# ribal-aladeeb/reinforcement-learning-2048

Hardware: AMD Instinct MI355X
Metric: 2048 env steps/sec + DQN updates/sec at 64k parallel boards, 1→8 MI355X (higher is better)
Workload: dtype u8

## Files before the change

### reinforcement-learning-2048_amd/csrc/g2048_conv64.hip

```cpp
#include <hip/hip_runtime.h>
#include <math.h>
#include <stdint.h>
#include <stdlib.h>

#include <mutex>
#include <unordered_map>

#include "../../include/g2048.h"
#include "g2048_board.hpp"
#include "g2048_common.hpp"

namespace {

typedef double d4 __attribute__((ext_vector_type(4)));

constexpr int NT = 256;
constexpr int TB = 16;
constexpr int XS = 17;
constexpr int DSB = 66;
constexpr int DPL = TB * DSB;
constexpr int HS = 258;
constexpr int H3S = 66;
constexpr int MAX_WG = 256;

constexpr int P_W1 = 0, P_B1 = 256, P_W2 = 320, P_B2 = 16704, P_F1 = 16768, P_FB1 = 33152,
              P_F2 = 33216, P_FB2 = 33472, P_N = 33476;
constexpr int SLAB = P_N + 4;
constexpr int FC_D2_LO = P_F1 / 2, FC_D2_HI = P_N / 2 + 1, FC_D2 = FC_D2_HI - FC_D2_LO;
constexpr int SHADOW_MIN_GRID = (FC_D2 + 63) / 64;
static_assert(P_F1 % 2 == 0 && P_N % 2 == 0 && SLAB % 2 == 0, "double2 ranges");
constexpr int PACK = 16384;
constexpr int PACKU = 9 * 4096;
constexpr int O_U_ON = 0, O_F1_ON = PACKU, O_U_TG = PACKU + PACK, O_F1_TG = 2 * PACKU + PACK,
              O_F1B = 2 * PACKU + 2 * PACK, O_UB = 2 * PACKU + 3 * PACK,
              PACK_ALL = 3 * PACKU + 3 * PACK, PACK_FWD = PACKU + PACK;
static_assert(PACK_ALL % 256 == 0 && PACK_FWD % 256 == 0, "pack grid");
constexpr int WS_STEP = PACK_ALL, WS_SLAB = PACK_ALL + 32;

#ifdef G2048_PHASE_PROF
__device__ unsigned long long g_cphase[32];
__shared__ unsigned long long g_lph[24];
#define CPHASE_INIT()                                                     \
    do {                                                                  \
        if (threadIdx.x == 0) {                                           \
            for (int k_ = 0; k_ < 23; ++k_) g_lph[k_] = 0ull;             \
            g_lph[23] = __builtin_amdgcn_s_memtime();                     \
        }                                                                 \
    } while (0)
#define CPHASE(k)                                                         \
    do {                                                                  \
        if (__builtin_amdgcn_readfirstlane(threadIdx.x) < 64) {           \
            const unsigned long long n_ = __builtin_amdgcn_s_memtime();   \
            if ((k) >= 0) g_lph[(k) < 0 ? 0 : (k)] += n_ - g_lph[23];     \
            g_lph[23] = n_;                                               \
        }                                                                 \
    } while (0)
#define CPHASE_FLUSH()                                                    \
    do {                                                                  \
        if (blockIdx.x == 0 && threadIdx.x == 0)                          \
            for (int k_ = 0; k_ < 23; ++k_) atomicAdd(&g_cphase[k_], g_lph[k_]); \
    } while (0)
#else
#define CPHASE_INIT()
#define CPHASE(k)
#define CPHASE_FLUSH()
#endif

typedef __attribute__((address_space(1))) const double gdouble;
__device__ __forceinline__ const gdouble* opaque(const double* p) {
    const gdouble* g = (const gdouble*)p;
    asm volatile("" : "+s"(g));
    return g;
}

__device__ __forceinline__ d4 mfma(double a, double b, d4 c) {
    return __builtin_amdgcn_mfma_f64_16x16x4f64(a, b, c, 0, 0, 0);
}

struct Net {
    const double *w1, *b1, *w2, *b2, *f1, *fb1, *f2, *fb2;
};

struct Packed {
    const double *u, *pf1;
};

struct SmallW {
    double w1[256], b1[64], b2[64], fb1[64], f2[256], fb2[4];
};

struct alignas(16) Smem {
    double x[TB * XS];
    double d[9 * DPL];
    double h2[TB * HS];
    double h3[TB * H3S];
    SmallW sw[2];
    double q[TB * 4];
    double q2[TB * 4];
    double y[TB];
    double r[TB];
    double dq[TB];
    double loss[TB];
    double f2p[4 * TB * 4];
    float disc[TB];
    int act[TB];
};

__device__ __forceinline__ void put_row(double* xr, uint4 v) {
    const uint32_t w[4] = {v.x, v.y, v.z, v.w};
#pragma unroll
    for (int k = 0; k < 4; ++k) {
        xr[4 * k + 0] = (double)(w[k] & 0xFFu);
        xr[4 * k + 1] = (double)((w[k] >> 8) & 0xFFu);
        xr[4 * k + 2] = (double)((w[k] >> 16) & 0xFFu);
        xr[4 * k + 3] = (double)(w[k] >> 24);
    }
}

__device__ __forceinline__ void stage_small(SmallW& W, const Net& n) {
    const int t = threadIdx.x;
    if (t >= 256) return;
    W.w1[t] = n.w1[t];
    W.f2[t] = n.f2[t];
    if (t < 64) {
        W.b1[t] = n.b1[t];
        W.b2[t] = n.b2[t];
        W.fb1[t] = n.fb1[t];
    }
    if (t < 4) W.fb2[t] = n.fb2[t];
}

template <bool WINO>
__device__ __forceinline__ uint64_t conv1_mfma(const double* xs, double* dst, const SmallW& W) {
    const int t = threadIdx.x, l = t & 63, w = t >> 6, lr = l & 15, lk = l >> 4;
    const int c = 16 * w + lr;
    const double wb = W.w1[c * 4 + lk];
    const int toff = (lk >> 1) * 4 + (lk & 1);
    const double* xr = xs + lr * XS + toff;
    d4 dq[9];
#pragma unroll
    for (int q = 0; q < 9; ++q)
        dq[q] = mfma(xr[(q / 3) * 4 + (q % 3)], wb, d4{0.0, 0.0, 0.0, 0.0});
    const double bc = W.b1[c];
    uint64_t mask = 0;
#pragma unroll
    for (int r = 0; r < 4; ++r) {
        double d[9];
#pragma unroll
        for (int q = 0; q < 9; ++q) {
            const double a = dq[q][r] + bc;
            d[q] = a > 0.0 ? a : 0.0;
            mask |= (uint64_t)(a > 0.0) << (9 * r + q);
        }
        double* out = dst + (4 * r + lk) * DSB + c;
        if constexpr (WINO) {
            double u[9];
#pragma unroll
            for (int x = 0; x < 3; ++x) {
                u[x] = d[x] - d[3 + x];
                u[3 + x] = d[3 + x];
                u[6 + x] = d[6 + x] - d[3 + x];
            }
#pragma unroll
            for (int y = 0; y < 3; ++y) {
                out[(3 * y + 0) * DPL] = u[3 * y] - u[3 * y + 1];
                out[(3 * y + 1) * DPL] = u[3 * y + 1];
                out[(3 * y + 2) * DPL] = u[3 * y + 2] - u[3 * y + 1];
            }
        } else {
#pragma unroll
            for (int q = 0; q < 9; ++q) out[q * DPL] = d[q];
        }
    }
    return mask;
}

__device__ __forceinline__ int pos_of(int p, int tap) {
    return ((p >> 1) + (tap >> 1)) * 3 + (p & 1) + (tap & 1);
}

__device__ void forward(Smem& M, const SmallW& W, const Packed& pk, double* q) {
    const int t = threadIdx.x, l = t & 63, w = t >> 6;
    const int lr = l & 15, lk = l >> 4;
    const gdouble* bp = opaque(pk.u) + (size_t)w * 9 * 16 * 64 + l;
    auto ld9 = [&](double(&b)[9], int s) {
#pragma unroll
        for (int x = 0; x < 9; ++x) b[x] = bp[(x * 16 + s) * 64];
    };
    double bb[3][9];
    ld9(bb[0], 0);
    ld9(bb[1], 1);
    __syncthreads();
    conv1_mfma<true>(M.x, M.d, W);
    __syncthreads();
    CPHASE(3);
    const gdouble* bpf = opaque(pk.pf1) + (size_t)w * 64 * 64 + l;
    auto ld8 = [&](double(&b)[8], int k) {
#pragma unroll
        for (int u = 0; u < 8; ++u) b[u] = bpf[(8 * k + u) * 64];
    };
    double bf[3][8];
    {
        d4 acc[9];
#pragma unroll
        for (int x = 0; x < 9; ++x) acc[x] = d4{0.0, 0.0, 0.0, 0.0};
        auto la9 = [&](double(&a)[9], int s) {
            const double* vr = M.d + lr * DSB + 4 * s + lk;
#pragma unroll
            for (int x = 0; x < 9; ++x) a[x] = vr[x * DPL];
        };
        double aa[2][9];
        la9(aa[0], 0);
#pragma unroll
        for (int s = 0; s < 16; ++s) {
            la9(aa[s & 1], s);
            if (s + 2 < 16) ld9(bb[(s + 2) % 3], s + 2);
#pragma unroll
            for (int x = 0; x < 9; ++x) acc[x] = mfma(aa[s & 1][x], bb[s % 3][x], acc[x]);
            __builtin_amdgcn_sched_barrier(0);
        }
        ld8(bf[0], 0);
        ld8(bf[1], 1);
        __builtin_amdgcn_sched_barrier(0);
        const int o = 16 * w + lr;
        const double bo = W.b2[o];
#pragma unroll
        for (int r = 0; r < 4; ++r) {
            double n[6];
#pragma unroll
            for (int x = 0; x < 3; ++x) {
                n[x] = acc[x][r] + acc[3 + x][r];
                n[3 + x] = acc[3 + x][r] + acc[6 + x][r];
            }
            double* hr = M.h2 + (4 * r + lk) * HS + o * 4;
#pragma unroll
            for (int py = 0; py < 2; ++py) {
                const double z0 = (n[3 * py] + n[3 * py + 1]) + bo;
                const double z1 = (n[3 * py + 1] + n[3 * py + 2]) + bo;
                hr[2 * py] = z0 > 0.0 ? z0 : 0.0;
                hr[2 * py + 1] = z1 > 0.0 ? z1 : 0.0;
            }
        }
    }
    __syncthreads();
    CPHASE(4);
    {
        d4 acc[4];
#pragma unroll
        for (int c = 0; c < 4; ++c) acc[c] = d4{0.0, 0.0, 0.0, 0.0};
        auto la8 = [&](double(&a)[8], int k) {
#pragma unroll
            for (int u = 0; u < 8; ++u) a[u] = M.h2[lr * HS + 4 * (8 * k + u) + lk];
        };
        double aa[2][8];
        la8(aa[0], 0);
#pragma unroll
        for (int k = 0; k < 8; ++k) {
            if (k + 1 < 8) la8(aa[(k + 1) & 1], k + 1);
            if (k + 2 < 8) ld8(bf[(k + 2) % 3], k + 2);
#pragma unroll
            for (int u = 0; u < 8; ++u) acc[u & 3] = mfma(aa[k & 1][u], bf[k % 3][u], acc[u & 3]);
            __builtin_amdgcn_sched_barrier(0);
        }
        const int j = 16 * w + lr;
        const double bj = W.fb1[j];
#pragma unroll
        for (int r = 0; r < 4; ++r) {
            const double z = ((acc[0][r] + acc[1][r]) + (acc[2][r] + acc[3][r])) + bj;
            M.h3[(4 * r + lk) * H3S + j] = z > 0.0 ? z : 0.0;
        }
    }
    CPHASE(5);
    {
        __builtin_amdgcn_wave_barrier();
        d4 acc = d4{0.0, 0.0, 0.0, 0.0};
#pragma unroll
        for (int s = 0; s < 4; ++s) {
            const int j = 16 * w + 4 * s + lk;
            const double av = M.h3[lr * H3S + j];
            const double bv = lr < 4 ? W.f2[lr * 64 + j] : 0.0;
            acc = mfma(av, bv, acc);
        }
        if (lr < 4) {
#pragma unroll
            for (int r = 0; r < 4; ++r) M.f2p[(w * TB + 4 * r + lk) * 4 + lr] = acc[r];
        }
    }
    __syncthreads();
    if (t < TB * 4) {
        const double* p = M.f2p + t;
        q[t] = ((p[0] + p[TB * 4]) + (p[2 * TB * 4] + p[3 * TB * 4])) + W.fb2[t & 3];
    }
    __syncthreads();
    CPHASE(6);
}

__device__ __forceinline__ int64_t sample_row(int64_t b, unsigned long long ep,
                                              unsigned long long count, uint32_t lo, uint32_t hi) {
    const uint4 u = g2048::philox10(
        make_uint4((uint32_t)b, (uint32_t)((uint64_t)b >> 32), (uint32_t)ep,
                   (uint32_t)(ep >> 32) | (g2048::DOMAIN_SAMPLE << 30)),
        lo, hi);
    return (int64_t)__umul64hi(((unsigned long long)u.y << 32) | u.x, count);
}

struct Ring {
    const uint4 *s, *s2;
    const uint8_t *a, *d;
    const int32_t* r;
    const unsigned long long* count;
};

struct PackArgs {
    const double *w2_on, *f1_on, *w2_tg, *f1_tg;
    double* out;
};

__device__ __forceinline__ double wino_u(double g0, double g1, double g2, double g3, int xi) {
    const int xy = xi / 3, xx = xi % 3;
    const double r0 = xy == 0 ? g0 : xy == 1 ? g0 + g2 : g2;
    const double r1 = xy == 0 ? g1 : xy == 1 ? g1 + g3 : g3;
    return xx == 0 ? r0 : xx == 1 ? r0 + r1 : r1;
}

__device__ __forceinline__ int idx_u(int o, int c, int xi) {
    return (((o >> 4) * 9 + xi) * 16 + (c >> 2)) * 64 + (c & 3) * 16 + (o & 15);
}
__device__ __forceinline__ int idx_ub(int o, int c, int xi) {
    return (((c >> 4) * 9 + xi) * 16 + (o >> 2)) * 64 + (o & 3) * 16 + (c & 15);
}
__device__ __forceinline__ int idx_pf1(int j, int k) {
    return ((j >> 4) * 64 + (k >> 2)) * 64 + (k & 3) * 16 + (j & 15);
}
__device__ __forceinline__ int idx_f1b(int j, int k) {
    return (((k >> 6) * 4 + ((k >> 4) & 3)) * 16 + (j >> 2)) * 64 + (j & 3) * 16 + (k & 15);
}

template <bool BWD>
__device__ __forceinline__ double pack_u(const double* w2, int i) {
    const int l = i & 63, lr = l & 15, lk = l >> 4;
    const int s = (i >> 6) & 15, xi = (i >> 10) % 9, w = (i >> 10) / 9;
    const int o = BWD ? 4 * s + lk : 16 * w + lr, c = BWD ? 16 * w + lr : 4 * s + lk;
    const double* g = w2 + o * 256 + c * 4;
    return wino_u(g[0], g[1], g[2], g[3], xi);
}

__device__ __forceinline__ double pack_f1(const double* f1, int i) {
    const int l = i & 63, lr = l & 15, lk = l >> 4;
    const int s = (i >> 6) & 63, w = i >> 12;
    return f1[(16 * w + lr) * 256 + 4 * s + lk];
}

__global__ __launch_bounds__(NT) void k_pack(PackArgs A) {
    const int e = blockIdx.x * NT + threadIdx.x;
    double v;
    if (e < O_F1_ON) {
        v = pack_u<false>(A.w2_on, e);
    } else if (e < O_U_TG) {
        v = pack_f1(A.f1_on, e - O_F1_ON);
    } else if (e < O_F1_TG) {
        v = pack_u<false>(A.w2_tg, e - O_U_TG);
    } else if (e < O_F1B) {
        v = pack_f1(A.f1_tg, e - O_F1_TG);
    } else if (e < O_UB) {
        const int i = e - O_F1B;
        const int l = i & 63, lr = l & 15, lk = l >> 4;
        const int s = (i >> 6) & 15, q = (i >> 10) & 3, w = i >> 12;
        v = A.f1_on[(4 * s + lk) * 256 + 64 * w + 16 * q + lr];
    } else {
        v = pack_u<true>(A.w2_on, e - O_UB);
    }
    A.out[e] = v;
}

struct TgtArgs {
    Net on, tg;
    Packed pon, ptg;
    Ring R;
    const unsigned long long* step;
    const int64_t* idx_in;
    int64_t batch;
    uint32_t seed_lo, seed_hi;
    float gamma;
    int double_dqn;
    int64_t* idx_out;
    double* y_out;
    unsigned long long* step_next;
};

struct TrainArgs {
    Net on;
    Packed pon;
    const double* pf1b;
    const double* p2b;
    Ring R;
    const int64_t* idx;
    const double* y;
    int64_t batch;
    double* dz2;
    double* slab;
    double* pre;
    double* h2g;
    double* dz3g;
};

struct FusedArgs {
    TgtArgs T;
    TrainArgs A;
};

template <bool GW>
__global__ __launch_bounds__(NT) void k_conv64_train_a(FusedArgs F) {
    __shared__ Smem M;
    const TgtArgs& T = F.T;
    const TrainArgs& A = F.A;
    const int t = threadIdx.x, l = t & 63, w = t >> 6;
    const int lr = l & 15, lk = l >> 4;
    d4 gf1[16];
#pragma unroll
    for (int c = 0; c < 16; ++c) gf1[c] = d4{0.0, 0.0, 0.0, 0.0};
    double gf2 = 0.0, gfb2 = 0.0, gfb1 = 0.0, gloss = 0.0;
    const unsigned long long ep = T.idx_in ? 0ull : *T.step;
    const unsigned long long count = T.idx_in ? 0ull : *T.R.count;
    if (blockIdx.x == 0 && t == 0) *T.step_next = *T.step + 1ull;
    CPHASE_INIT();
    const SmallW& W = M.sw[0];
    const int64_t ntiles = (A.batch + TB - 1) / TB;
    uint4 s2v = make_uint4(0u, 0u, 0u, 0u), sv = s2v;
    double rj = 0.0;
    float disc = 0.f;
    int aj = 0;
    auto fetch = [&](int64_t tile) {
        s2v = sv = make_uint4(0u, 0u, 0u, 0u);
        rj = 0.0;
        disc = 0.f;
        aj = 0;
        const int64_t b = tile * TB + t;
        if (t < TB && tile < ntiles && b < A.batch) {
            const int64_t row =
                T.idx_in ? T.idx_in[b] : sample_row(b, ep, count, T.seed_lo, T.seed_hi);
            T.idx_out[b] = row;
            s2v = T.R.s2[row];
            sv = T.R.s[row];
            rj = (double)T.R.r[row];
            disc = (float)(1 - (int)T.R.d[row]) * T.gamma;
            aj = T.R.a[row];
        }
    };
    fetch(blockIdx.x);
    stage_small(M.sw[0], A.on);
    stage_small(M.sw[1], T.tg);
    for (int64_t tile = blockIdx.x; tile < ntiles; tile += gridDim.x) {
        const int64_t b0 = tile * TB;
        __syncthreads();
        const uint4 s_cur = sv;
        const int a_cur = aj;
        if (t < TB) {
            put_row(M.x + t * XS, s2v);
            M.r[t] = rj;
            M.disc[t] = disc;
        }
        CPHASE(1);
#pragma unroll 1
        for (int k = T.double_dqn ? 0 : 1; k < 3; ++k) {
            if (k == 2) {
                if (t < TB) {
                    double yv = 0.0;
                    if (b0 + t < A.batch) {
                        const double* qt = M.q + t * 4;
                        double next;
                        if (T.double_dqn) {
                            const double* qo = M.q2 + t * 4;
                            next = qt[g2048::argmax4_torch(qo[0], qo[1], qo[2], qo[3])];
                        } else {
                            next = g2048::qmax4_torch(qt[0], qt[1], qt[2], qt[3]);
                        }
                        {
#pragma clang fp contract(off)
                            yv = M.r[t] + (double)M.disc[t] * next;
                        }
                        T.y_out[b0 + t] = yv;
                    }
                    M.y[t] = yv;
                    put_row(M.x + t * XS, s_cur);
                    M.act[t] = a_cur;
                }
                CPHASE(2);
            }
            forward(M, M.sw[k == 1 ? 1 : 0], k == 1 ? T.ptg : T.pon, k == 0 ? M.q2 : M.q);
        }
        fetch(tile + gridDim.x);
        CPHASE(8);
        if (t < TB) {
            double dq = 0.0, ls = 0.0;
            if (b0 + t < A.batch) {
#pragma clang fp contract(off)
                const double e = M.q[t * 4 + M.act[t]] - M.y[t];
                dq = 2.0 * e;
                ls = e * e;
            }
            M.dq[t] = dq;
            M.loss[t] = ls;
        }
        __syncthreads();
        {
            double acc = 0.0, accb = 0.0;
            for (int s = 0; s < TB; ++s) {
                if (M.act[s] == w) {
                    acc = fma(M.dq[s], M.h3[s * H3S + l], acc);
                    accb += M.dq[s];
                }
            }
            gf2 += acc;
            if (l == 0) gfb2 += accb;
        }
        if (t == 0) {
            double ls = 0.0;
            for (int s = 0; s < TB; ++s) ls += M.loss[s];
            gloss += ls;
        }
        __syncthreads();
        CPHASE(9);
#pragma unroll
        for (int bb = 0; bb < 4; ++bb) {
            const int s = 4 * w + bb;
            double& hv = M.h3[s * H3S + l];
            hv = hv > 0.0 ? M.dq[s] * W.f2[M.act[s] * 64 + l] : 0.0;
        }
        __syncthreads();
        if (t < 64) {
            double acc = 0.0;
            for (int s = 0; s < TB; ++s) acc += M.h3[s * H3S + t];
            gfb1 += acc;
        }
        CPHASE(10);
        if constexpr (GW) {
            const int64_t rb0 = b0 * 256;
#pragma unroll
            for (int k = 0; k < 8; ++k) {
                const int e = 2 * (t + NT * k);
                const int bq = e >> 8, col = e & 255;
                *reinterpret_cast<double2*>(A.h2g + rb0 + e) =
                    make_double2(M.h2[bq * HS + col], M.h2[bq * HS + col + 1]);
            }
#pragma unroll
            for (int k = 0; k < 2; ++k) {
                const int e = 2 * (t + NT * k);
                const int bq = e >> 6, col = e & 63;
                *reinterpret_cast<double2*>(A.dz3g + b0 * 64 + e) =
                    make_double2(M.h3[bq * H3S + col], M.h3[bq * H3S + col + 1]);
            }
        }
#ifndef G2048_TIMING_NO_WGRAD
#pragma unroll
        for (int s = 0; s < 4 && !GW; ++s) {
            double op[17];
            op[0] = M.h3[(4 * s + lk) * H3S + 16 * w + lr];
#pragma unroll
            for (int cb = 0; cb < 16; ++cb) op[1 + cb] = M.h2[(4 * s + lk) * HS + 16 * cb + lr];
            __builtin_amdgcn_sched_barrier(0);
#pragma unroll
            for (int cb = 0; cb < 16; ++cb) gf1[cb] = mfma(op[0], op[1 + cb], gf1[cb]);
            __builtin_amdgcn_sched_barrier(0);
        }
#endif
        CPHASE(11);
        {
            d4 acc[4];
#pragma unroll
            for (int c = 0; c < 4; ++c) acc[c] = d4{0.0, 0.0, 0.0, 0.0};
            const gdouble* bp = opaque(A.pf1b) + (size_t)w * 4 * 16 * 64 + l;
            auto ld4 = [&](double(&b)[4], int s) {
#pragma unroll
                for (int cb = 0; cb < 4; ++cb) b[cb] = bp[(cb * 16 + s) * 64];
            };
            double ah[16];
#pragma unroll
            for (int s = 0; s < 16; ++s) ah[s] = M.h3[lr * H3S + 4 * s + lk];
            auto mm4 = [&](const double(&b)[4], int s) {
#pragma unroll
                for (int cb = 0; cb < 4; ++cb) acc[cb] = mfma(ah[s], b[cb], acc[cb]);
            };
            double bb[3][4];
            ld4(bb[0], 0);
            ld4(bb[1], 1);
#pragma unroll
            for (int s = 0; s < 16; ++s) {
                if (s + 2 < 16) ld4(bb[(s + 2) % 3], s + 2);
                mm4(bb[s % 3], s);
                __builtin_amdgcn_sched_barrier(0);
            }
#pragma unroll
            for (int cb = 0; cb < 4; ++cb)
#pragma unroll
                for (int r = 0; r < 4; ++r) {
                    const int bq = 4 * r + lk, k = 64 * w + 16 * cb + lr;
                    A.dz2[(b0 + bq) * 256 + k] = M.h2[bq * HS + k] > 0.0 ? acc[cb][r] : 0.0;
                }
        }
        CPHASE(12);
    }
    double* sl = A.slab + (int64_t)blockIdx.x * SLAB;
#ifndef G2048_TIMING_NO_WGRAD
    if constexpr (!GW) {
#pragma unroll
        for (int cb = 0; cb < 16; ++cb)
#pragma unroll
            for (int r = 0; r < 4; ++r)
                sl[P_F1 + (16 * w + 4 * r + lk) * 256 + 16 * cb + lr] = gf1[cb][r];
    }
#endif
    if (t < 64) sl[P_FB1 + t] = gfb1;
    sl[P_F2 + w * 64 + l] = gf2;
    if (l == 0) sl[P_FB2 + w] = gfb2;
    if (t == 0) sl[P_N] = gloss;
    CPHASE(13);
    CPHASE_FLUSH();
}

constexpr int NT8 = 512;

__device__ __forceinline__ void conv1_v8(const double* xs, double* dst, const SmallW& W) {
    const int t = threadIdx.x, l = t & 63, w = t >> 6, cw = w & 3, hw = w >> 2;
    const int lr = l & 15, lk = l >> 4;
    const int c = 16 * cw + lr;
    const double wb = W.w1[c * 4 + lk];
    const int toff = (lk >> 1) * 4 + (lk & 1);
    const double* xr = xs + lr * XS + toff;
    d4 dq[9];
#pragma unroll
    for (int q = 0; q < 9; ++q)
        dq[q] = mfma(xr[(q / 3) * 4 + (q % 3)], wb, d4{0.0, 0.0, 0.0, 0.0});
    const double bc = W.b1[c];
#pragma unroll
    for (int rr = 0; rr < 2; ++rr) {
        double d[9];
#pragma unroll
        for (int q = 0; q < 9; ++q) {
            const double a = (hw ? dq[q][2 + rr] : dq[q][rr]) + bc;
            d[q] = a > 0.0 ? a : 0.0;
        }
        double* out = dst + (4 * (2 * hw + rr) + lk) * DSB + c;
        double u[9];
#pragma unroll
        for (int x = 0; x < 3; ++x) {
            u[x] = d[x] - d[3 + x];
            u[3 + x] = d[3 + x];
            u[6 + x] = d[6 + x] - d[3 + x];
        }
#pragma unroll
        for (int y = 0; y < 3; ++y) {
            out[(3 * y + 0) * DPL] = u[3 * y] - u[3 * y + 1];
            out[(3 * y + 1) * DPL] = u[3 * y + 1];
            out[(3 * y + 2) * DPL] = u[3 * y + 2] - u[3 * y + 1];
        }
    }
}

template <int P0, int NP>
__device__ __forceinline__ void conv2_ldb(const gdouble* bp, double (&b)[5], int s) {
#pragma unroll
    for (int x = 0; x < NP; ++x) b[x] = bp[((P0 + x) * 16 + s) * 64];
}

template <int P0, int NP>
__device__ __forceinline__ void conv2_half(const Smem& M, const gdouble* bp, double (&bb)[2][5],
                                           d4 (&acc)[5]) {
    const int l = threadIdx.x & 63, lr = l & 15, lk = l >> 4;
#pragma unroll
    for (int x = 0; x < 5; ++x) acc[x] = d4{0.0, 0.0, 0.0, 0.0};
    auto la = [&](double(&a)[5], int s) {
        const double* vr = M.d + lr * DSB + 4 * s + lk;
#pragma unroll
        for (int x = 0; x < NP; ++x) a[x] = vr[(P0 + x) * DPL];
    };
    double aa[2][5];
    la(aa[0], 0);
#pragma unroll
    for (int s = 0; s < 16; ++s) {
        if (s + 1 < 16) {
            la(aa[(s + 1) & 1], s + 1);
            conv2_ldb<P0, NP>(bp, bb[(s + 1) & 1], s + 1);
        }
#pragma unroll
        for (int x = 0; x < NP; ++x) acc[x] = mfma(aa[s & 1][x], bb[s & 1][x], acc[x]);
        __builtin_amdgcn_sched_barrier(0);
    }
}

template <int P0, int NP>
__device__ __forceinline__ void conv2_put(double* dst, const d4 (&acc)[5], int o) {
    const int lk = (threadIdx.x & 63) >> 4;
#pragma unroll
    for (int x = 0; x < NP; ++x)
#pragma unroll
        for (int r = 0; r < 4; ++r) dst[(P0 + x) * DPL + (4 * r + lk) * DSB + o] = acc[x][r];
}

__device__ void forward8(Smem& M, const SmallW& W, const Packed& pk, double* q) {
    const int t = threadIdx.x, l = t & 63, w = t >> 6, cw = w & 3, hw = w >> 2;
    const int lr = l & 15, lk = l >> 4;
    const gdouble* bp = opaque(pk.u) + (size_t)cw * 9 * 16 * 64 + l;
    __syncthreads();
    conv1_v8(M.x, M.d, W);
    double bb[2][5];
    if (hw)
        conv2_ldb<5, 4>(bp, bb[0], 0);
    else
        conv2_ldb<0, 5>(bp, bb[0], 0);
    __syncthreads();
    CPHASE(3);
    const gdouble* bpf = opaque(pk.pf1) + (size_t)cw * 64 * 64 + l;
    const int u0 = 2 * hw;
    auto ld4f = [&](double(&b)[4], int k) {
        b[0] = bpf[(8 * k + u0) * 64];
        b[1] = bpf[(8 * k + u0 + 1) * 64];
        b[2] = bpf[(8 * k + u0 + 4) * 64];
        b[3] = bpf[(8 * k + u0 + 5) * 64];
    };
    double bf[3][4];
    d4 acc[5];
    if (hw)
        conv2_half<5, 4>(M, bp, bb, acc);
    else
        conv2_half<0, 5>(M, bp, bb, acc);
    ld4f(bf[0], 0);
    ld4f(bf[1], 1);
    __builtin_amdgcn_sched_barrier(0);
    const int o = 16 * cw + lr;
    __syncthreads();
    if (hw)
        conv2_put<5, 4>(M.d, acc, o);
    else
        conv2_put<0, 5>(M.d, acc, o);
    __syncthreads();
    {
        const double bo = W.b2[o];
#pragma unroll
        for (int rr = 0; rr < 2; ++rr) {
            const int b = 4 * (2 * hw + rr) + lk;
            const double* mr = M.d + b * DSB + o;
            double m[9];
#pragma unroll
            for (int x = 0; x < 9; ++x) m[x] = mr[x * DPL];
            double n[6];
#pragma unroll
            for (int x = 0; x < 3; ++x) {
                n[x] = m[x] + m[3 + x];
                n[3 + x] = m[3 + x] + m[6 + x];
            }
            double* hr = M.h2 + b * HS + o * 4;
#pragma unroll
            for (int py = 0; py < 2; ++py) {
                const double z0 = (n[3 * py] + n[3 * py + 1]) + bo;
                const double z1 = (n[3 * py + 1] + n[3 * py + 2]) + bo;
                hr[2 * py] = z0 > 0.0 ? z0 : 0.0;
                hr[2 * py + 1] = z1 > 0.0 ? z1 : 0.0;
            }
        }
    }
    __syncthreads();
    CPHASE(4);
    {
        d4 fa[2] = {d4{0.0, 0.0, 0.0, 0.0}, d4{0.0, 0.0, 0.0, 0.0}};
        auto la4 = [&](double(&a)[4], int k) {
            const double* hr = M.h2 + lr * HS + 4 * (8 * k) + lk;
            a[0] = hr[4 * u0];
            a[1] = hr[4 * (u0 + 1)];
            a[2] = hr[4 * (u0 + 4)];
            a[3] = hr[4 * (u0 + 5)];
        };
        double aa[2][4];
        la4(aa[0], 0);
#pragma unroll
        for (int k = 0; k < 8; ++k) {
            if (k + 1 < 8) la4(aa[(k + 1) & 1], k + 1);
            if (k + 2 < 8) ld4f(bf[(k + 2) % 3], k + 2);
            const double(&a)[4] = aa[k & 1];
            const double(&b)[4] = bf[k % 3];
            fa[0] = mfma(a[0], b[0], fa[0]);
            fa[1] = mfma(a[1], b[1], fa[1]);
            fa[0] = mfma(a[2], b[2], fa[0]);
            fa[1] = mfma(a[3], b[3], fa[1]);
            __builtin_amdgcn_sched_barrier(0);
        }
        const d4 part = fa[0] + fa[1];
        double* xch = M.d + (size_t)(cw * 64 + l) * 4;
        if (hw) {
#pragma unroll
            for (int r = 0; r < 4; ++r) xch[r] = part[r];
        }
        __syncthreads();
        if (!hw) {
            const int j = 16 * cw + lr;
            const double bj = W.fb1[j];
#pragma unroll
            for (int r = 0; r < 4; ++r) {
                const double z = (part[r] + xch[r]) + bj;
                M.h3[(4 * r + lk) * H3S + j] = z > 0.0 ? z : 0.0;
            }
        }
    }
    CPHASE(5);
    if (!hw) {
        __builtin_amdgcn_wave_barrier();
        d4 a2 = d4{0.0, 0.0, 0.0, 0.0};
#pragma unroll
        for (int s = 0; s < 4; ++s) {
            const int j = 16 * cw + 4 * s + lk;
            const double av = M.h3[lr * H3S + j];
            const double bv = lr < 4 ? W.f2[lr * 64 + j] : 0.0;
            a2 = mfma(av, bv, a2);
        }
        if (lr < 4) {
#pragma unroll
            for (int r = 0; r < 4; ++r) M.f2p[(cw * TB + 4 * r + lk) * 4 + lr] = a2[r];
        }
    }
    __syncthreads();
    if (t < TB * 4) {
        const double* p = M.f2p + t;
        q[t] = ((p[0] + p[TB * 4]) + (p[2 * TB * 4] + p[3 * TB * 4])) + W.fb2[t & 3];
    }
    __syncthreads();
    CPHASE(6);
}

__global__ __launch_bounds__(NT8) void k_conv64_train_a8(FusedArgs F) {
    __shared__ Smem M;
    const TgtArgs& T = F.T;
    const TrainArgs& A = F.A;
    const int t = threadIdx.x, l = t & 63, w = t >> 6, cw = w & 3, hw = w >> 2;
    const int lr = l & 15, lk = l >> 4;
    d4 gf1[8];
#pragma unroll
    for (int c = 0; c < 8; ++c) gf1[c] = d4{0.0, 0.0, 0.0, 0.0};
    double gf2 = 0.0, gfb2 = 0.0, gfb1 = 0.0, gloss = 0.0;
    const unsigned long long ep = T.idx_in ? 0ull : *T.step;
    const unsigned long long count = T.idx_in ? 0ull : *T.R.count;
    if (blockIdx.x == 0 && t == 0) *T.step_next = *T.step + 1ull;
    CPHASE_INIT();
    const SmallW& W = M.sw[0];
    const int64_t ntiles = (A.batch + TB - 1) / TB;
    uint4 s2v = make_uint4(0u, 0u, 0u, 0u), sv = s2v;
    double rj = 0.0;
    float disc = 0.f;
    int aj = 0;
    auto fetch = [&](int64_t tile) {
        s2v = sv = make_uint4(0u, 0u, 0u, 0u);
        rj = 0.0;
        disc = 0.f;
        aj = 0;
        const int64_t b = tile * TB + t;
        if (t < TB && tile < ntiles && b < A.batch) {
            const int64_t row =
                T.idx_in ? T.idx_in[b] : sample_row(b, ep, count, T.seed_lo, T.seed_hi);
            T.idx_out[b] = row;
            s2v = T.R.s2[row];
            sv = T.R.s[row];
            rj = (double)T.R.r[row];
            disc = (float)(1 - (int)T.R.d[row]) * T.gamma;
            aj = T.R.a[row];
        }
    };
    fetch(blockIdx.x);
    stage_small(M.sw[0], A.on);
    stage_small(M.sw[1], T.tg);
    for (int64_t tile = blockIdx.x; tile < ntiles; tile += gridDim.x) {
        const int64_t b0 = tile * TB;
        __syncthreads();
        const uint4 s_cur = sv;
        const int a_cur = aj;
        if (t < TB) {
            put_row(M.x + t * XS, s2v);
            M.r[t] = rj;
            M.disc[t] = disc;
        }
        CPHASE(1);
#pragma unroll 1
        for (int k = T.double_dqn ? 0 : 1; k < 3; ++k) {
            if (k == 2) {
                if (t < TB) {
                    double yv = 0.0;
                    if (b0 + t < A.batch) {
                        const double* qt = M.q + t * 4;
                        double next;
                        if (T.double_dqn) {
                            const double* qo = M.q2 + t * 4;
                            next = qt[g2048::argmax4_torch(qo[0], qo[1], qo[2], qo[3])];
                        } else {
                            next = g2048::qmax4_torch(qt[0], qt[1], qt[2], qt[3]);
                        }
                        {
#pragma clang fp contract(off)
                            yv = M.r[t] + (double)M.disc[t] * next;
                        }
                        T.y_out[b0 + t] = yv;
                    }
                    M.y[t] = yv;
                    put_row(M.x + t * XS, s_cur);
                    M.act[t] = a_cur;
                }
                CPHASE(2);
            }
            forward8(M, M.sw[k == 1 ? 1 : 0], k == 1 ? T.ptg : T.pon, k == 0 ? M.q2 : M.q);
        }
        fetch(tile + gridDim.x);
        CPHASE(8);
        if (t < TB) {
            double dq = 0.0, ls = 0.0;
            if (b0 + t < A.batch) {
#pragma clang fp contract(off)
                const double e = M.q[t * 4 + M.act[t]] - M.y[t];
                dq = 2.0 * e;
                ls = e * e;
            }
            M.dq[t] = dq;
            M.loss[t] = ls;
        }
        __syncthreads();
        if (t < 256) {
            double acc = 0.0, accb = 0.0;
            for (int s = 0; s < TB; ++s) {
                if (M.act[s] == w) {
                    acc = fma(M.dq[s], M.h3[s * H3S + l], acc);
                    accb += M.dq[s];
                }
            }
            gf2 += acc;
            if (l == 0) gfb2 += accb;
        }
        if (t == 0) {
            double ls = 0.0;
            for (int s = 0; s < TB; ++s) ls += M.loss[s];
            gloss += ls;
        }
        __syncthreads();
        CPHASE(9);
#pragma unroll
        for (int bb = 0; bb < 2; ++bb) {
            const int s = 2 * w + bb;
            double& hv = M.h3[s * H3S + l];
            hv = hv > 0.0 ? M.dq[s] * W.f2[M.act[s] * 64 + l] : 0.0;
        }
        __syncthreads();
        if (t < 64) {
            double acc = 0.0;
            for (int s = 0; s < TB; ++s) acc += M.h3[s * H3S + t];
            gfb1 += acc;
        }
        CPHASE(10);
#pragma unroll
        for (int s = 0; s < 4; ++s) {
            double op[9];
            op[0] = M.h3[(4 * s + lk) * H3S + 16 * cw + lr];
#pragma unroll
            for (int cb = 0; cb < 8; ++cb)
                op[1 + cb] = M.h2[(4 * s + lk) * HS + 16 * (8 * hw + cb) + lr];
            __builtin_amdgcn_sched_barrier(0);
#pragma unroll
            for (int cb = 0; cb < 8; ++cb) gf1[cb] = mfma(op[0], op[1 + cb], gf1[cb]);
            __builtin_amdgcn_sched_barrier(0);
        }
        CPHASE(11);
        {
            d4 acc[2] = {d4{0.0, 0.0, 0.0, 0.0}, d4{0.0, 0.0, 0.0, 0.0}};
            const gdouble* bp = opaque(A.pf1b) + (size_t)w * 2 * 16 * 64 + l;
            auto ld2 = [&](double(&b)[2], int s) {
                b[0] = bp[s * 64];
                b[1] = bp[(16 + s) * 64];
            };
            double ah[16];
#pragma unroll
            for (int s = 0; s < 16; ++s) ah[s] = M.h3[lr * H3S + 4 * s + lk];
            double bb[3][2];
            ld2(bb[0], 0);
            ld2(bb[1], 1);
#pragma unroll
            for (int s = 0; s < 16; ++s) {
                if (s + 2 < 16) ld2(bb[(s + 2) % 3], s + 2);
                acc[0] = mfma(ah[s], bb[s % 3][0], acc[0]);
                acc[1] = mfma(ah[s], bb[s % 3][1], acc[1]);
                __builtin_amdgcn_sched_barrier(0);
            }
#pragma unroll
            for (int cb = 0; cb < 2; ++cb)
#pragma unroll
                for (int r = 0; r < 4; ++r) {
                    const int bq = 4 * r + lk, kk = 32 * w + 16 * cb + lr;
                    A.dz2[(b0 + bq) * 256 + kk] = M.h2[bq * HS + kk] > 0.0 ? acc[cb][r] : 0.0;
                }
        }
        CPHASE(12);
    }
    double* sl = A.slab + (int64_t)blockIdx.x * SLAB;
#pragma unroll
    for (int cb = 0; cb < 8; ++cb)
#pragma unroll
        for (int r = 0; r < 4; ++r)
            sl[P_F1 + (16 * cw + 4 * r + lk) * 256 + 16 * (8 * hw + cb) + lr] = gf1[cb][r];
    if (t < 64) sl[P_FB1 + t] = gfb1;
    if (t < 256) sl[P_F2 + w * 64 + l] = gf2;
    if (t < 256 && l == 0) sl[P_FB2 + w] = gfb2;
    if (t == 0) sl[P_N] = gloss;
    CPHASE(13);
    CPHASE_FLUSH();
}

struct alignas(16) SmemB {
    double x[TB * XS];
    double d[9 * DPL];
    double dm[9 * DPL];
    SmallW sw;
};

template <bool GW>
__global__ __launch_bounds__(NT) void k_conv64_train_b(TrainArgs A) {
    __shared__ SmemB M;
    const int t = threadIdx.x, l = t & 63, w = t >> 6;
    const int lr = l & 15, lk = l >> 4;
    g2048::SlabShadow<double2, 8> sh;
    const int chunk = (FC_D2 + (int)gridDim.x - 1) / (int)gridDim.x;
    const int d2 = FC_D2_LO + (int)blockIdx.x * chunk + l;
    const bool sh_on = A.pre != nullptr && l < chunk && d2 < FC_D2_HI;
    if (A.pre)
        sh.init(sh_on ? reinterpret_cast<const double2*>(A.slab) + d2 : nullptr, SLAB / 2,
                (int)gridDim.x, w);
    d4 gw2[16];
#pragma unroll
    for (int c = 0; c < 16; ++c) gw2[c] = d4{0.0, 0.0, 0.0, 0.0};
    double gw1[4] = {0.0, 0.0, 0.0, 0.0}, gb1 = 0.0, gb2 = 0.0;
    CPHASE_INIT();
    const int64_t ntiles = (A.batch + TB - 1) / TB;
    uint4 sv = make_uint4(0u, 0u, 0u, 0u);
    double2 zv[4][2];
    auto fetch = [&](int64_t tile) {
        sv = make_uint4(0u, 0u, 0u, 0u);
        const int64_t b = tile * TB + t;
        if (t < TB && tile < ntiles && b < A.batch) sv = A.R.s[A.idx[b]];
#pragma unroll
        for (int k = 0; k < 4; ++k) {
            zv[k][0] = zv[k][1] = make_double2(0.0, 0.0);
            if (tile < ntiles) {
                const double2* src = reinterpret_cast<const double2*>(
                    A.dz2 + (tile * TB + (t >> 6) + 4 * k) * 256 + (t & 63) * 4);
                zv[k][0] = src[0];
                zv[k][1] = src[1];
            }
        }
    };
    fetch(blockIdx.x);
    stage_small(M.sw, A.on);
    for (int64_t tile = blockIdx.x; tile < ntiles; tile += gridDim.x) {
        __syncthreads();
        if (t < TB) put_row(M.x + t * XS, sv);
        {
            const int o = t & 63;
#pragma unroll
            for (int k = 0; k < 4; ++k) {
                const double y00 = zv[k][0].x, y01 = zv[k][0].y, y10 = zv[k][1].x, y11 = zv[k][1].y;
                gb2 += ((y00 + y01) + y10) + y11;
                const double m[9] = {y00, y00 + y01, y01, y00 + y10, ((y00 + y01) + y10) + y11,
                                     y01 + y11, y10, y10 + y11, y11};
                double* dst = M.dm + ((t >> 6) + 4 * k) * DSB + o;
#pragma unroll
                for (int x = 0; x < 9; ++x) dst[x * DPL] = m[x];
            }
        }
        CPHASE(14);
        __syncthreads();
        const uint64_t mask = conv1_mfma<false>(M.x, M.d, M.sw);
        __syncthreads();
        fetch(tile + gridDim.x);
        CPHASE(15);
        auto lds17 = [&](double(&v)[17], int s) {
            const int p = s >> 2, bq = 4 * (s & 3) + lk;
            const int xc = (p >> 1) * 6 + (p & 1) * 2;
            v[0] = M.dm[xc * DPL + bq * DSB + 16 * w + lr];
#pragma unroll
            for (int tap = 0; tap < 4; ++tap) {
                const double* dr = M.d + pos_of(p, tap) * DPL + bq * DSB + lr;
#pragma unroll
                for (int cb = 0; cb < 4; ++cb) v[1 + tap * 4 + cb] = dr[16 * cb];
            }
        };
#ifndef G2048_TIMING_NO_WGRAD
#pragma unroll 4
        for (int s = 0; s < 16 && !GW; ++s) {
            if (A.pre && (s & 3) == 0) sh.issue<0>();
            double op[17];
            lds17(op, s);
            __builtin_amdgcn_sched_barrier(0);
#pragma unroll
            for (int k = 0; k < 16; ++k) gw2[k] = mfma(op[0], op[1 + k], gw2[k]);
            __builtin_amdgcn_sched_barrier(0);
            if (A.pre && (s & 3) == 3) sh.consume<0>();
        }
#endif
        CPHASE(16);
        d4 dv[9];
#pragma unroll
        for (int x = 0; x < 9; ++x) dv[x] = d4{0.0, 0.0, 0.0, 0.0};
        {
            const gdouble* ub = opaque(A.p2b) + (size_t)w * 9 * 16 * 64 + l;
            auto ld9 = [&](double(&b)[9], int s) {
#pragma unroll
                for (int x = 0; x < 9; ++x) b[x] = ub[(x * 16 + s) * 64];
            };
            double bb[3][9];
            ld9(bb[0], 0);
            ld9(bb[1], 1);
            auto la9 = [&](double(&a)[9], int s) {
                const double* ar = M.dm + lr * DSB + 4 * s + lk;
#pragma unroll
                for (int x = 0; x < 9; ++x) a[x] = ar[x * DPL];
            };
            double aa[2][9];
#pragma unroll
            for (int s = 0; s < 16; ++s) {
                la9(aa[s & 1], s);
                if (s + 2 < 16) ld9(bb[(s + 2) % 3], s + 2);
#pragma unroll
                for (int x = 0; x < 9; ++x) dv[x] = mfma(aa[s & 1][x], bb[s % 3][x], dv[x]);
                __builtin_amdgcn_sched_barrier(0);
            }
        }
        CPHASE(17);
        {
#pragma unroll
            for (int r = 0; r < 4; ++r) {
                double u[9];
#pragma unroll
                for (int x = 0; x < 3; ++x) {
                    u[x] = dv[x][r];
                    u[3 + x] = (dv[3 + x][r] - dv[x][r]) - dv[6 + x][r];
                    u[6 + x] = dv[6 + x][r];
                }
                double dz[9];
#pragma unroll
                for (int y = 0; y < 3; ++y) {
                    dz[3 * y] = u[3 * y];
                    dz[3 * y + 1] = (u[3 * y + 1] - u[3 * y]) - u[3 * y + 2];
                    dz[3 * y + 2] = u[3 * y + 2];
                }
                const double* xr = M.x + (4 * r + lk) * XS;
#pragma unroll
                for (int q = 0; q < 9; ++q) {
                    const double z = (mask >> (9 * r + q)) & 1ull ? dz[q] : 0.0;
                    const int i0 = (q / 3) * 4 + (q % 3);
                    gw1[0] = fma(z, xr[i0], gw1[0]);
                    gw1[1] = fma(z, xr[i0 + 1], gw1[1]);
                    gw1[2] = fma(z, xr[i0 + 4], gw1[2]);
                    gw1[3] = fma(z, xr[i0 + 5], gw1[3]);
                    gb1 += z;
                }
            }
        }
        CPHASE(18);
    }
    {
        double* sl = A.slab + (int64_t)blockIdx.x * SLAB;
#ifdef G2048_TIMING_NO_WGRAD
        if (A.batch < 0)
#else
        if (!GW)
#endif
#pragma unroll
        for (int cb = 0; cb < 4; ++cb)
#pragma unroll
            for (int r = 0; r < 4; ++r) {
                const int64_t e = (P_W2 + (16 * w + 4 * r + lk) * 256 + (16 * cb + lr) * 4) / 2;
                g2048::slab_store16(reinterpret_cast<double2*>(sl), e,
                                    make_double2(gw2[cb][r], gw2[4 + cb][r]));
                g2048::slab_store16(reinterpret_cast<double2*>(sl), e + 1,
                                    make_double2(gw2[8 + cb][r], gw2[12 + cb][r]));
            }
    }
#ifndef G2048_TIMING_NO_WGRAD
    if (A.pre) {
#else
    if (A.pre && A.batch < 0) {
#endif
        while (sh.pending()) {
            sh.issue<0>();
            sh.consume<0>();
        }
    }
    double* sl = A.slab + (int64_t)blockIdx.x * SLAB;
    __syncthreads();
    double* red = M.d;
#pragma unroll
    for (int k = 0; k < 4; ++k) red[k * 256 + t] = gw1[k];
    red[4 * 256 + t] = gb1;
    red[5 * 256 + t] = gb2;
    __syncthreads();
    if (t < 64) {
        const int c = t, ww = c >> 4, cl = c & 15;
        const int base = ww * 64 + cl;
#pragma unroll
        for (int k = 0; k < 5; ++k) {
            const double* v = red + k * 256 + base;
            const double sm = ((v[0] + v[16]) + v[32]) + v[48];
            if (k < 4) sl[P_W1 + c * 4 + k] = sm;
            else sl[P_B1 + c] = sm;
        }
        const double* v2 = red + 5 * 256 + c;
        sl[P_B2 + c] = ((v2[0] + v2[64]) + v2[128]) + v2[192];
    }
    if (A.pre) {
        __shared__ double2 part[3][64];
        if (w > 0) part[w - 1][l] = sh.acc;
        __syncthreads();
        if (w == 0 && sh_on) {
            const double2 a = sh.acc, b = part[0][l], c = part[1][l], d = part[2][l];
            reinterpret_cast<double2*>(A.pre)[d2] =
                make_double2(((a.x + b.x) + c.x) + d.x, ((a.y + b.y) + c.y) + d.y);
        }
    }
    CPHASE(19);
    CPHASE_FLUSH();
}

constexpr int WKR = 64;
constexpr int WAS = 66;
constexpr int WG_MAX_SPLIT = 48;
constexpr int WG_BLOCK = 4096;

struct WgSplit {
    int s1, s2;
};
WgSplit wgrad_splits(int64_t batch) {
    const int64_t st_f = (batch + 63) / 64, st_w = (batch + 15) / 16;
    const int s1 = (int)(st_f < 12 ? st_f : 12);
    const int64_t s2 = 4 * (int64_t)s1 < st_w ? 4 * s1 : st_w;
    return WgSplit{s1, (int)s2};
}
int64_t wgrad_part_doubles(int64_t batch) {
    const WgSplit sp = wgrad_splits(batch);
    return (int64_t)4 * (sp.s1 + sp.s2) * WG_BLOCK;
}

struct WgArgs {
    const double *w1, *b1;
    const uint4* s;
    const int64_t* idx;
    const double* dz2;
    const double* h2;
    const double* dz3;
    int64_t batch;
    int s1, s2;
    int64_t chunk1, chunk2;
    double* part;
};

constexpr int NTW = 512;
using WgTile = double[WKR][WAS];

template <bool CW>
__device__ __forceinline__ void wgrad_block(const WgArgs& A, WgTile* As, WgTile* Bs, int unit,
                                            int split) {
    const int t = threadIdx.x, l = t & 63, w = t >> 6, lr = l & 15, lk = l >> 4;
    const bool stager = w >= 4;
    const int wr = w & 3, pt = t & 255;
    const int64_t chunk = CW ? A.chunk2 : A.chunk1;
    const int64_t k0 = (int64_t)split * chunk;
    const int64_t k1 = k0 + chunk < A.batch ? k0 + chunk : A.batch;
    constexpr int SPB = CW ? 16 : 64;
    const int c = 16 * wr + lr;
    const double wb = CW && stager ? A.w1[c * 4 + lk] : 0.0, bc = CW && stager ? A.b1[c] : 0.0;
    const int col = pt & 63;
    uint64_t blo = 0, bhi = 0;
    int64_t ridx = -1;
    double ga[16], gb[16];
#define WG_FETCH(st0_)                                                                        \
    do {                                                                                      \
        const int64_t st0f = (st0_);                                                          \
        if (CW) {                                                                             \
            blo = 0, bhi = 0;                                                                 \
            if (ridx >= 0) {                                                                  \
                const uint4 v = A.s[ridx];                                                    \
                blo = (uint64_t)v.x | ((uint64_t)v.y << 32);                                  \
                bhi = (uint64_t)v.z | ((uint64_t)v.w << 32);                                  \
            }                                                                                 \
            const int64_t nb0 = st0f + SPB + lr;                                              \
            ridx = nb0 < k1 ? A.idx[nb0] : -1;                                                \
            _Pragma("unroll") for (int k = 0; k < 4; ++k) {                                   \
                const int64_t b = st0f + (pt >> 6) + 4 * k;                                   \
                double2 p0 = make_double2(0.0, 0.0), p1 = p0;                                 \
                if (b < k1) {                                                                 \
                    const double2* src =                                                      \
                        reinterpret_cast<const double2*>(A.dz2 + b * 256 + col * 4);          \
                    p0 = src[0];                                                              \
                    p1 = src[1];                                                              \
                }                                                                             \
                ga[4 * k] = p0.x, ga[4 * k + 1] = p0.y, ga[4 * k + 2] = p1.x,                 \
                ga[4 * k + 3] = p1.y;                                                         \
            }                                                                                 \
        } else {                                                                              \
            _Pragma("unroll") for (int k = 0; k < 16; ++k) {                                  \
                const int64_t b = st0f + (pt >> 6) + 4 * k;                                   \
                const bool ok = b < k1;                                                       \
                ga[k] = ok ? A.dz3[b * 64 + col] : 0.0;                                       \
                gb[k] = ok ? A.h2[b * 256 + 64 * unit + col] : 0.0;                           \
            }                                                                                 \
        }                                                                                     \
    } while (0)
#define WG_PUT(bf_)                                                                           \
    do {                                                                                      \
        WgTile& At = As[(bf_)];                                                               \
        WgTile& Bt = Bs[(bf_)];                                                               \
        if (CW) {                                                                             \
            _Pragma("unroll") for (int k = 0; k < 4; ++k)                                     \
                _Pragma("unroll") for (int p = 0; p < 4; ++p)                                 \
                    At[((pt >> 6) + 4 * k) * 4 + p][col] = ga[4 * k + p];                     \
            _Pragma("unroll") for (int p = 0; p < 4; ++p) {                                   \
                const int q = pos_of(p, unit);                                                \
                const int rr = q / 3 + (lk >> 1), cc = q % 3 + (lk & 1);                      \
                const uint64_t half = rr >= 2 ? bhi : blo;                                    \
                const double xv =                                                             \
                    (double)((uint32_t)(half >> (8 * (4 * (rr & 1) + cc))) & 0xFFu);          \
                const d4 dq = mfma(xv, wb, d4{0.0, 0.0, 0.0, 0.0});                           \
                _Pragma("unroll") for (int r = 0; r < 4; ++r) {                               \
                    const double a = dq[r] + bc;                                              \
                    Bt[(4 * r + lk) * 4 + p][c] = a > 0.0 ? a : 0.0;                          \
                }                                                                             \
            }                                                                                 \
        } else {                                                                              \
            _Pragma("unroll") for (int k = 0; k < 16; ++k) {                                  \
                At[(pt >> 6) + 4 * k][col] = ga[k];                                           \
                Bt[(pt >> 6) + 4 * k][col] = gb[k];                                           \
            }                                                                                 \
        }                                                                                     \
    } while (0)
    if (stager && k0 < k1) {
        if (CW) ridx = k0 + lr < k1 ? A.idx[k0 + lr] : -1;
        WG_FETCH(k0);
        WG_PUT(0);
        if (k0 + SPB < k1) WG_FETCH(k0 + SPB);
    }
    __syncthreads();
    d4 acc[4];
#pragma unroll
    for (int nb = 0; nb < 4; ++nb) acc[nb] = d4{0.0, 0.0, 0.0, 0.0};
    int bf = 0;
    for (int64_t st0 = k0; st0 < k1; st0 += SPB, bf ^= 1) {
        if (!stager) {
            const WgTile& At = As[bf];
            const WgTile& Bt = Bs[bf];
#pragma unroll
            for (int s4 = 0; s4 < WKR / 4; ++s4) {
                const int kr = 4 * s4 + lk;
                const double av = At[kr][16 * wr + lr];
                double bv[4];
#pragma unroll
                for (int nb = 0; nb < 4; ++nb) bv[nb] = Bt[kr][16 * nb + lr];
#ifndef G2048_TIMING_WG_NOGEMM
#pragma unroll
                for (int nb = 0; nb < 4; ++nb) acc[nb] = mfma(av, bv[nb], acc[nb]);
#else
                acc[0][0] += av + bv[0] + bv[1] + bv[2] + bv[3];
#endif
            }
        }
#ifndef G2048_TIMING_WG_NOPUT
        else if (st0 + SPB < k1) {
            WG_PUT(bf ^ 1);
            if (st0 + 2 * SPB < k1) WG_FETCH(st0 + 2 * SPB);
        }
#endif
        __syncthreads();
    }
#undef WG_FETCH
#undef WG_PUT
    if (stager) return;
    const int64_t slot =
        CW ? (int64_t)unit * A.s2 + split : (int64_t)4 * A.s2 + unit * A.s1 + split;
    double* out = A.part + slot * WG_BLOCK;
#pragma unroll
    for (int nb = 0; nb < 4; ++nb)
#pragma unroll
        for (int r = 0; r < 4; ++r) out[(16 * wr + 4 * r + lk) * 64 + 16 * nb + lr] = acc[nb][r];
}

__global__ __launch_bounds__(NTW) void k_conv64_wgrad(WgArgs A) {
    __shared__ WgTile As[2];
    __shared__ WgTile Bs[2];
    const int nw2 = 4 * A.s2;
    if ((int)blockIdx.x < nw2)
        wgrad_block<true>(A, As, Bs, (int)blockIdx.x / A.s2, (int)blockIdx.x % A.s2);
    else
        wgrad_block<false>(A, As, Bs, ((int)blockIdx.x - nw2) / A.s1,
                           ((int)blockIdx.x - nw2) % A.s1);
}

constexpr int RW = 16;
static_assert(MAX_WG % RW == 0 && SLAB % 2 == 0, "reduction: MAX_WG / RW slabs per wave, pairs");

struct RedArgs {
    const double* slab;
    const double* pre;
    int nslab;
    double* grad;
    double* loss;
    const unsigned long long* step_next;
    unsigned long long* step;
    double* p[8];
    double* tp[8];
    unsigned long long sync_every;
    double *m, *v;
    double lr, b1, b2, eps;
    int adam;
    double* pk;
    const double* part;
    int nsplit1, nsplit2;
};

__global__ __launch_bounds__(64 * RW) void k_conv64_reduce(RedArgs A) {
    __shared__ double2 part[RW][64];
    const int lane = threadIdx.x & 63, wave = threadIdx.x >> 6;
    const int pos = blockIdx.x * 128 + 2 * lane;
    const int base[8] = {P_W1, P_B1, P_W2, P_B2, P_F1, P_FB1, P_F2, P_FB2};
    double am[2] = {0.0, 0.0}, av[2] = {0.0, 0.0}, ap[2] = {0.0, 0.0};
    int kk[2] = {0, 0};
    unsigned long long tt = 0;
    g2048::Adam64Coef cf{0.0, 0.0};
    if (A.adam && wave == 0) {
        tt = *A.step_next;
#pragma unroll
        for (int h = 0; h < 2; ++h) {
            const int ps = pos + h;
            if (ps >= P_N) continue;
            int k = 7;
            while (ps < base[k]) --k;
            kk[h] = k;
            am[h] = A.m[ps];
            av[h] = A.v[ps];
            ap[h] = A.p[k][ps - base[k]];
        }
    }
    const bool summed = A.pre != nullptr && pos >= P_F1;
    const double2 pv = (summed && wave == 0 && pos <= P_N)
                           ? *reinterpret_cast<const double2*>(A.pre + pos)
                           : make_double2(0.0, 0.0);
    double2 r = make_double2(0.0, 0.0);
    const bool gw_w2 = A.part != nullptr && pos >= P_W2 && pos < P_B2;
    const bool gw_f1 = A.part != nullptr && pos >= P_F1 && pos < P_FB1;
    if (gw_w2) {
        const int i = pos - P_W2, o = i >> 8, cc = (i >> 2) & 63, tap = i & 3;
#pragma unroll
        for (int h = 0; h < WG_MAX_SPLIT / RW; ++h) {
            const int sp = wave + RW * h;
            if (sp >= A.nsplit2) break;
            r.x += A.part[((int64_t)tap * A.nsplit2 + sp) * WG_BLOCK + o * 64 + cc];
            r.y += A.part[((int64_t)(tap + 1) * A.nsplit2 + sp) * WG_BLOCK + o * 64 + cc];
        }
    } else if (gw_f1) {
        const int i = pos - P_F1, j = i >> 8, k = i & 255;
#pragma unroll
        for (int h = 0; h < WG_MAX_SPLIT / RW; ++h) {
            const int sp = wave + RW * h;
            if (sp >= A.nsplit1) break;
            const double2 v = *reinterpret_cast<const double2*>(
                A.part + ((int64_t)4 * A.nsplit2 + (k >> 6) * A.nsplit1 + sp) * WG_BLOCK +
                j * 64 + (k & 63));
            r.x += v.x;
            r.y += v.y;
        }
    } else
#ifdef G2048_TIMING_NO_WGRAD
    if (pos <= P_N && !summed && !(pos >= P_W2 && pos < P_B2)) {
#else
    if (pos <= P_N && !summed) {
#endif
        double2 v[MAX_WG / RW];
#pragma unroll
        for (int k = 0; k < MAX_WG / RW; ++k) {
            const int g = wave + RW * k;
            v[k] = g < A.nslab ? *reinterpret_cast<const double2*>(A.slab + (int64_t)g * SLAB + pos)
                               : make_double2(0.0, 0.0);
// ... 412 lines not shown
```

Baseline: 170.9 billion.

## Parameterize prefetch depths and overlap last-tile work with gradient flush

```diff
diff --git a/reinforcement-learning-2048_amd/csrc/g2048_conv64.hip b/reinforcement-learning-2048_amd/csrc/g2048_conv64.hip
--- a/reinforcement-learning-2048_amd/csrc/g2048_conv64.hip
+++ b/reinforcement-learning-2048_amd/csrc/g2048_conv64.hip
@@ -73,6 +73,19 @@
     return g;
 }
 
+#ifndef G2048_CONV2_DEPTH
+#define G2048_CONV2_DEPTH 2
+#endif
+#ifndef G2048_DV_DEPTH
+#define G2048_DV_DEPTH 2
+#endif
+#ifndef G2048_DH2_DEPTH
+#define G2048_DH2_DEPTH 2
+#endif
+constexpr int C2D = G2048_CONV2_DEPTH, DVD = G2048_DV_DEPTH, DHD = G2048_DH2_DEPTH;
+static_assert(C2D >= 2 && C2D <= 6 && DVD >= 2 && DVD <= 6 && DHD >= 2 && DHD <= 15,
+              "prefetch depths: at most 63 loads in flight (vmcnt)");
+
 __device__ __forceinline__ d4 mfma(double a, double b, d4 c) {
     return __builtin_amdgcn_mfma_f64_16x16x4f64(a, b, c, 0, 0, 0);
 }
@@ -187,9 +200,9 @@
 #pragma unroll
         for (int x = 0; x < 9; ++x) b[x] = bp[(x * 16 + s) * 64];
     };
-    double bb[3][9];
-    ld9(bb[0], 0);
-    ld9(bb[1], 1);
+    double bb[C2D + 1][9];
+#pragma unroll
+    for (int s = 0; s < C2D; ++s) ld9(bb[s], s);
     __syncthreads();
     conv1_mfma<true>(M.x, M.d, W);
     __syncthreads();
@@ -214,14 +227,14 @@
 #pragma unroll
         for (int s = 0; s < 16; ++s) {
             la9(aa[s & 1], s);
-            if (s + 2 < 16) ld9(bb[(s + 2) % 3], s + 2);
-#pragma unroll
-            for (int x = 0; x < 9; ++x) acc[x] = mfma(aa[s & 1][x], bb[s % 3][x], acc[x]);
+            if (s + C2D < 16) ld9(bb[(s + C2D) % (C2D + 1)], s + C2D);
+            if (s == 16 - C2D) ld8(bf[0], 0);
+            if (s == 17 - C2D) ld8(bf[1], 1);
+#pragma unroll
+            for (int x = 0; x < 9; ++x)
+                acc[x] = mfma(aa[s & 1][x], bb[s % (C2D + 1)][x], acc[x]);
             __builtin_amdgcn_sched_barrier(0);
         }
-        ld8(bf[0], 0);
-        ld8(bf[1], 1);
-        __builtin_amdgcn_sched_barrier(0);
         const int o = 16 * w + lr;
         const double bo = W.b2[o];
 #pragma unroll
@@ -450,6 +463,35 @@
     fetch(blockIdx.x);
     stage_small(M.sw[0], A.on);
     stage_small(M.sw[1], T.tg);
+    const gdouble* bph = nullptr;
+    auto ld4 = [&](double(&b)[4], int s) {
+#pragma unroll
+        for (int cb = 0; cb < 4; ++cb) b[cb] = bph[(cb * 16 + s) * 64];
+    };
+    double bh[DHD + 1][4];
+    auto dh2 = [&](int64_t b0) {
+        d4 acc[4];
+#pragma unroll
+        for (int c = 0; c < 4; ++c) acc[c] = d4{0.0, 0.0, 0.0, 0.0};
+        double ah[16];
+#pragma unroll
+        for (int s = 0; s < 16; ++s) ah[s] = M.h3[lr * H3S + 4 * s + lk];
+#pragma unroll
+        for (int s = 0; s < 16; ++s) {
+            if (s + DHD < 16) ld4(bh[(s + DHD) % (DHD + 1)], s + DHD);
+#pragma unroll
+            for (int cb = 0; cb < 4; ++cb) acc[cb] = mfma(ah[s], bh[s % (DHD + 1)][cb], acc[cb]);
+            __builtin_amdgcn_sched_barrier(0);
+        }
+#pragma unroll
+        for (int cb = 0; cb < 4; ++cb)
+#pragma unroll
+            for (int r = 0; r < 4; ++r) {
+                const int bq = 4 * r + lk, k = 64 * w + 16 * cb + lr;
+                A.dz2[(b0 + bq) * 256 + k] = M.h2[bq * HS + k] > 0.0 ? acc[cb][r] : 0.0;
+            }
+    };
+    int64_t b_last = -1;
     for (int64_t tile = blockIdx.x; tile < ntiles; tile += gridDim.x) {
         const int64_t b0 = tile * TB;
         __syncthreads();
@@ -551,6 +593,9 @@
                     make_double2(M.h3[bq * H3S + col], M.h3[bq * H3S + col + 1]);
             }
         }
+        bph = opaque(A.pf1b) + (size_t)w * 4 * 16 * 64 + l;
+#pragma unroll
+        for (int s = 0; s < DHD; ++s) ld4(bh[s], s);
 #ifndef G2048_TIMING_NO_WGRAD
 #pragma unroll
         for (int s = 0; s < 4 && !GW; ++s) {
@@ -565,39 +610,10 @@
         }
 #endif
         CPHASE(11);
-        {
-            d4 acc[4];
-#pragma unroll
-            for (int c = 0; c < 4; ++c) acc[c] = d4{0.0, 0.0, 0.0, 0.0};
-            const gdouble* bp = opaque(A.pf1b) + (size_t)w * 4 * 16 * 64 + l;
-            auto ld4 = [&](double(&b)[4], int s) {
-#pragma unroll
-                for (int cb = 0; cb < 4; ++cb) b[cb] = bp[(cb * 16 + s) * 64];
-            };
-            double ah[16];
-#pragma unroll
-            for (int s = 0; s < 16; ++s) ah[s] = M.h3[lr * H3S + 4 * s + lk];
-            auto mm4 = [&](const double(&b)[4], int s) {
-#pragma unroll
-                for (int cb = 0; cb < 4; ++cb) acc[cb] = mfma(ah[s], b[cb], acc[cb]);
-            };
-            double bb[3][4];
-            ld4(bb[0], 0);
-            ld4(bb[1], 1);
-#pragma unroll
-            for (int s = 0; s < 16; ++s) {
-                if (s + 2 < 16) ld4(bb[(s + 2) % 3], s + 2);
-                mm4(bb[s % 3], s);
-                __builtin_amdgcn_sched_barrier(0);
-            }
-#pragma unroll
-            for (int cb = 0; cb < 4; ++cb)
-#pragma unroll
-                for (int r = 0; r < 4; ++r) {
-                    const int bq = 4 * r + lk, k = 64 * w + 16 * cb + lr;
-                    A.dz2[(b0 + bq) * 256 + k] = M.h2[bq * HS + k] > 0.0 ? acc[cb][r] : 0.0;
-                }
-        }
+        if (tile + gridDim.x < ntiles)
+            dh2(b0);
+        else
+            b_last = b0;
         CPHASE(12);
     }
     double* sl = A.slab + (int64_t)blockIdx.x * SLAB;
@@ -610,6 +626,7 @@
                 sl[P_F1 + (16 * w + 4 * r + lk) * 256 + 16 * cb + lr] = gf1[cb][r];
     }
 #endif
+    if (b_last >= 0) dh2(b_last);
     if (t < 64) sl[P_FB1 + t] = gfb1;
     sl[P_F2 + w * 64 + l] = gf2;
     if (l == 0) sl[P_FB2 + w] = gfb2;
@@ -1051,6 +1068,16 @@
     };
     fetch(blockIdx.x);
     stage_small(M.sw, A.on);
+    double* const slw = A.slab + (int64_t)blockIdx.x * SLAB;
+    auto store_w2 = [&](int j) {
+        const int cb = j >> 2, r = j & 3;
+        const int64_t e = (P_W2 + (16 * w + 4 * r + lk) * 256 + (16 * cb + lr) * 4) / 2;
+        g2048::slab_store16(reinterpret_cast<double2*>(slw), e,
+                            make_double2(gw2[cb][r], gw2[4 + cb][r]));
+        g2048::slab_store16(reinterpret_cast<double2*>(slw), e + 1,
+                            make_double2(gw2[8 + cb][r], gw2[12 + cb][r]));
+    };
+    const bool have_last = (int64_t)blockIdx.x < ntiles;
     for (int64_t tile = blockIdx.x; tile < ntiles; tile += gridDim.x) {
         __syncthreads();
         if (t < TB) put_row(M.x + t * XS, sv);
@@ -1071,6 +1098,7 @@
         __syncthreads();
         const uint64_t mask = conv1_mfma<false>(M.x, M.d, M.sw);
         __syncthreads();
+        const bool last = tile + gridDim.x >= ntiles;
         fetch(tile + gridDim.x);
         CPHASE(15);
         auto lds17 = [&](double(&v)[17], int s) {
@@ -1086,7 +1114,7 @@
         };
 #ifndef G2048_TIMING_NO_WGRAD
 #pragma unroll 4
-        for (int s = 0; s < 16 && !GW; ++s) {
+        for (int s = 0; s < 16 && !GW && !last; ++s) {
             if (A.pre && (s & 3) == 0) sh.issue<0>();
             double op[17];
             lds17(op, s);
@@ -1107,9 +1135,9 @@
 #pragma unroll
                 for (int x = 0; x < 9; ++x) b[x] = ub[(x * 16 + s) * 64];
             };
-            double bb[3][9];
-            ld9(bb[0], 0);
-            ld9(bb[1], 1);
+            double bb[DVD + 1][9];
+#pragma unroll
+            for (int s = 0; s < DVD; ++s) ld9(bb[s], s);
             auto la9 = [&](double(&a)[9], int s) {
                 const double* ar = M.dm + lr * DSB + 4 * s + lk;
 #pragma unroll
@@ -1119,9 +1147,10 @@
 #pragma unroll
             for (int s = 0; s < 16; ++s) {
                 la9(aa[s & 1], s);
-                if (s + 2 < 16) ld9(bb[(s + 2) % 3], s + 2);
-#pragma unroll
-                for (int x = 0; x < 9; ++x) dv[x] = mfma(aa[s & 1][x], bb[s % 3][x], dv[x]);
+                if (s + DVD < 16) ld9(bb[(s + DVD) % (DVD + 1)], s + DVD);
+#pragma unroll
+                for (int x = 0; x < 9; ++x)
+                    dv[x] = mfma(aa[s & 1][x], bb[s % (DVD + 1)][x], dv[x]);
                 __builtin_amdgcn_sched_barrier(0);
             }
         }
@@ -1159,22 +1188,40 @@
         CPHASE(18);
     }
     {
-        double* sl = A.slab + (int64_t)blockIdx.x * SLAB;
 #ifdef G2048_TIMING_NO_WGRAD
         if (A.batch < 0)
 #else
         if (!GW)
 #endif
-#pragma unroll
-        for (int cb = 0; cb < 4; ++cb)
-#pragma unroll
-            for (int r = 0; r < 4; ++r) {
-                const int64_t e = (P_W2 + (16 * w + 4 * r + lk) * 256 + (16 * cb + lr) * 4) / 2;
-                g2048::slab_store16(reinterpret_cast<double2*>(sl), e,
-                                    make_double2(gw2[cb][r], gw2[4 + cb][r]));
-                g2048::slab_store16(reinterpret_cast<double2*>(sl), e + 1,
-                                    make_double2(gw2[8 + cb][r], gw2[12 + cb][r]));
-            }
+        {
+#pragma unroll
+            for (int cb = 0; cb < 4; ++cb) {
+#pragma unroll 1
+                for (int g = 0; g < 4 && have_last; ++g) {
+                    if (A.pre && cb == 0) sh.issue<0>();
+                    const int xc = (g >> 1) * 6 + (g & 1) * 2;
+                    double op[4][5];
+#pragma unroll
+                    for (int i = 0; i < 4; ++i) {
+                        const int bq = 4 * i + lk;
+                        op[i][0] = M.dm[xc * DPL + bq * DSB + 16 * w + lr];
+#pragma unroll
+                        for (int tap = 0; tap < 4; ++tap)
+                            op[i][1 + tap] = M.d[pos_of(g, tap) * DPL + bq * DSB + 16 * cb + lr];
+                    }
+                    __builtin_amdgcn_sched_barrier(0);
+#pragma unroll
+                    for (int i = 0; i < 4; ++i)
+#pragma unroll
+                        for (int tap = 0; tap < 4; ++tap)
+                            gw2[tap * 4 + cb] = mfma(op[i][0], op[i][1 + tap], gw2[tap * 4 + cb]);
+                    __builtin_amdgcn_sched_barrier(0);
+                    if (A.pre && cb == 0) sh.consume<0>();
+                }
+#pragma unroll
+                for (int r = 0; r < 4; ++r) store_w2(cb * 4 + r);
+            }
+        }
     }
 #ifndef G2048_TIMING_NO_WGRAD
     if (A.pre) {
```

Result: no change. 170.7 billion (-0.1%).
